# marella/ctransformers

Measured on NVIDIA H100. Metric: decode tokens/s Llama-2-7B Q4_K_M b=1, higher is better.
Workload: dtype int8 (q4_K/q6_K weights x q8_K activations, mma.sync u8 x s8 -> exact int32), fp32 combine in the reference's order

## Files before the change

ctransformers_b200/csrc/engine.cu:

```cuda
#include "engine.cuh"

#include <algorithm>
#include <chrono>
#include <cstdio>
#include <cstring>
#include <stdexcept>

#include "attention.cuh"
#include "matvec.cuh"
#include "prefill.cuh"
#include "repack.cuh"
#include "sample_gpu.cuh"
#include "stream.cuh"
#include "tables.hpp"
#include "tp_nccl.hpp"

namespace ctb {

#define CTB_CUDA(expr)                                                                                         \
  do {                                                                                                         \
    cudaError_t e__ = (expr);                                                                                  \
    if (e__ != cudaSuccess)                                                                                    \
      throw std::runtime_error(std::string("CUDA error: ") + cudaGetErrorString(e__) + " at " + __FILE__ + ":" + \
                               std::to_string(__LINE__) + " (" #expr ")" + watchdog_note());                   \
// ... 19 lines not shown
  int prev = -1;
  explicit DeviceGuard(int dev) {
    cudaGetDevice(&prev);
    if (prev != dev) {
      cudaError_t e = cudaSetDevice(dev);
      if (e != cudaSuccess) throw std::runtime_error(std::string("CUDA error: ") + cudaGetErrorString(e) + " (cudaSetDevice)");
    }
  }
  ~DeviceGuard() { int cur = -1; cudaGetDevice(&cur); if (prev >= 0 && cur != prev) cudaSetDevice(prev); }
};

struct StepOp {
  Phase ph;
  int mvk = 0;
  bool stream = false;
};

__global__ void k_advance(int* state, int* out_tokens) {
  const int t = state[4];
  out_tokens[state[2]] = t;
  state[0] = t;
  state[1] += 1;
  state[2] += 1;
  state[3] = state[1] + 1;
}

struct PrefillState {
  std::vector<void*> bufs;
  PPhase* d_prog = nullptr;
  int n_phases = 0;
// ... 20 lines not shown

size_t engine_arena_bytes(const GGUFFile& g, const HParams& hp) {
  size_t total = 0;
  for (const auto& t : g.tensors) {
    total += align_up(t.nbytes, 256) + 4 * 256;
    if (t.ne[1] > 0) total += align_up(t.nbytes / (size_t)t.ne[1] * ST_ROWS, 256);
  }
  total += UP_CHUNK * UP_BUFS + 256;
  const size_t kv = (size_t)hp.n_layer * (hp.n_ctx + 256) * hp.n_embd_gqa() * 2;
  total += 2 * align_up(kv, 256);
  total += 3 * align_up(65536 * 2, 256);
  total += align_up((size_t)hp.n_ctx * (hp.head_dim() / 2) * 8, 256);
  const size_t qkv = (size_t)hp.n_embd + 2 * (size_t)hp.n_embd_gqa();
  total += 4 * (2 * (size_t)hp.n_embd + qkv + 4 * (size_t)hp.n_embd + 2 * (size_t)hp.n_ff + 2 * (size_t)hp.n_vocab) + 64 * 256 + 8192;
  total += ((size_t)hp.n_layer * 10 + 8) * (sizeof(Phase) * 2 + 2 * 1024) + 8192;
  total += 1 << 20;
  return total;
}

void* Engine::alloc(size_t bytes, size_t align) {
  const size_t off = align_up(arena_used_, align);
  if (off + bytes > arena_size_) throw std::runtime_error("device arena exhausted");
  arena_used_ = off + bytes;
  return arena_ + off;
}

struct Uploader {
  uint8_t* host[UP_BUFS] = {nullptr, nullptr, nullptr};
  uint8_t* dev[UP_BUFS] = {nullptr, nullptr, nullptr};
  cudaEvent_t done[UP_BUFS] = {nullptr, nullptr, nullptr};
// ... 262 lines not shown
  }
  const size_t gqa_l = (size_t)nkv_ * hp_.head_dim(), qw_l = (size_t)nh_ * hp_.head_dim();
  const size_t kv = (size_t)hp_.n_layer * hp_.n_ctx * gqa_l;
  const size_t vv = (size_t)hp_.n_layer * kv_ctx_pad(hp_.n_ctx) * gqa_l;
  kc_ = (uint16_t*)alloc(kv * 2);
  vc_ = (uint16_t*)alloc(vv * 2);
  CTB_CUDA(cudaMemset(kc_, 0, kv * 2));
  CTB_CUDA(cudaMemset(vc_, 0, vv * 2));
  const size_t qkv = qw_l + 2 * gqa_l;
  d_state_ = (int*)alloc(64);
  xa_ = (float*)alloc(hp_.n_embd * 4); xb_ = (float*)alloc(hp_.n_embd * 4);
  qkv_ = (float*)alloc(qkv * 4);
  attn_ = (float*)alloc(hp_.n_embd * 4); attn_o_ = (float*)alloc(hp_.n_embd * 4);
  ffn_ = (float*)alloc((size_t)nff_ * 4);
  ffn2_ = (float*)alloc((size_t)nff_ * 4);
  d_logits_ = (float*)alloc((size_t)hp_.n_vocab * 4);
  d_embd_ = (float*)alloc(hp_.n_embd * 4);
  d_logits_keep_ = (float*)alloc((size_t)hp_.n_vocab * 4);
  d_embd_keep_ = (float*)alloc(hp_.n_embd * 4);
  d_sync_ = (unsigned*)alloc(64);
  CTB_CUDA(cudaMemset(d_state_, 0, 64));
  CTB_CUDA(cudaMemset(d_sync_, 0, 64));
  CTB_CUDA(cudaMallocHost(&h_logits_, (size_t)hp_.n_vocab * 4));
  CTB_CUDA(cudaMallocHost(&h_embd_, (size_t)hp_.n_embd * 4));
  memset(h_logits_, 0, (size_t)hp_.n_vocab * 4);
  memset(h_embd_, 0, (size_t)hp_.n_embd * 4);

  if (const char* e = getenv("CTB_NO_PDL")) pdl_ = !(e[0] == '1');
  if (const char* e = getenv("CTB_NO_SPEC")) spec_on_ = !(e[0] == '1');
  if (const char* e = getenv("CTB_STEP_FUSE")) fused_ = !(e[0] == '0');
// ... 142 lines not shown
    op.ph.em.out = buf; op.ph.em.K = n_embd;
    ops_.push_back(op);
  };
  auto take_input = [&](MVParams& p) {
    if (!xchg_due) return;
    p.x = (const float*)xc_ll_[tp_.rank]; p.x_mode = 2; p.x_parts = tp_.world; p.x_stride = n_embd; p.sum_out = x_sum_into;
  };
  auto mark_exchange = [&](size_t first_op) {
    if (!xchg_due) return;
    if (ops_.size() != first_op + 1) throw std::runtime_error("tensor parallel (fused exchange): the consumer of an exchange must be one mat-vec phase");
    fill_xc(ops_[first_op].ph.xc, 1);
    n_xchg++;
    xchg_due = false; x_sum_into = nullptr;
  };
  const float kq_scale = 1.0f / sqrtf((float)n_embd / (float)hp_.n_head);
  ops_.clear();
  {
    StepOp op{};
    op.ph.kind = PH_EMBED;
    op.ph.em.table = tok_embd_; op.ph.em.row_bytes = tok_row_bytes_; op.ph.em.tokens = d_state_; op.ph.em.out = xa_;
    op.ph.em.type = tok_type_; op.ph.em.K = n_embd; op.ph.em.n_vocab = hp_.n_vocab;
    ops_.push_back(op);
  }
  float* x = xa_;
  float* y = xb_;
  for (int il = 0; il < hp_.n_layer; il++) {
    const LayerW& L = layers_[il];
    uint16_t* kc = kc_ + (size_t)il * hp_.n_ctx * gqa;
    uint16_t* vc = vc_ + (size_t)il * gqa * kv_ctx_pad(hp_.n_ctx);
    AttnParams ap{};
// ... 22 lines not shown
          p.act = act_format_for(ws[i]->type); p.nseg = 0;
          for (int j = i; j < 3; j++)
            if (!done[j] && act_format_for(ws[j]->type) == p.act) { p.seg[p.nseg++] = seg(*ws[j], outs[j]); done[j] = true; }
          push_matvec(p, MVK_QKV);
        }
        mark_exchange(first_op);
      }
      push_attn();
      {
        MVParams p{};
        p.x = attn_; p.norm_mode = NORM_NONE; p.K = qw; p.act = act_format_for(L.wo.type); p.nseg = 1;
        p.seg[0] = (!tp || tp_lead) ? seg(L.wo, y, EPI_ADD, x) : seg(L.wo, y);
        push_matvec(p, MVK_WO);
        if (tp) push_xchg(y);
      }
      {
        MVParams p{};
        p.x = y; p.norm_w = L.ffn_norm; p.norm_mode = NORM_RMS; p.eps = hp_.eps; p.K = n_embd;
        const size_t first_op = ops_.size();
        take_input(p);
        p.act = act_format_for(L.w1.type); p.nseg = 2;
        p.seg[0] = seg(L.w1, ffn_, EPI_SILU); p.seg[1] = seg(L.w3, ffn2_);
        push_matvec(p, MVK_UP);
        mark_exchange(first_op);
      }
      {
        MVParams p{};
        p.x = ffn_; p.x2 = ffn2_; p.x_mode = 1; p.norm_mode = NORM_NONE; p.K = nff_; p.act = act_format_for(L.w2.type); p.nseg = 1;
        p.seg[0] = (!tp || tp_lead) ? seg(L.w2, x, EPI_ADD, y) : seg(L.w2, x);
        push_matvec(p, MVK_DOWN);
        if (tp) push_xchg(x);
      }
    } else {
      const int qkv_w = (hp_.n_head + 2 * n_kv) * hd;
      float* q = qkv_; float* k = qkv_ + (size_t)hp_.n_head * hd; float* v = k + (size_t)n_kv * hd;
      const bool two_norms = L.attn_norm2 != nullptr;
      const bool fuse = !two_norms && act_format_for(L.wqkv.type) == act_format_for(L.w3.type);
      {
        MVParams p{};
        p.x = x; p.norm_mode = NORM_LAYER; p.eps = hp_.eps; p.K = n_embd;
        p.norm_w = two_norms ? L.attn_norm2 : L.attn_norm; p.norm_b = two_norms ? L.attn_norm2_b : L.attn_norm_b;
        p.act = act_format_for(L.wqkv.type); p.nseg = 1;
        p.seg[0] = seg(L.wqkv, qkv_);
        if (fuse) { p.seg[1] = seg(L.w3, ffn_, EPI_GELU); p.nseg = 2; }
        ap.q = q; ap.k = k; ap.v = v; ap.q_stride = qkv_w; ap.kv_stride = qkv_w;
        push_matvec(p, MVK_QKV);
      }
      if (!fuse) {
        MVParams p{};
        p.x = x; p.norm_mode = NORM_LAYER; p.eps = hp_.eps; p.K = n_embd; p.norm_w = L.attn_norm; p.norm_b = L.attn_norm_b;
        p.act = act_format_for(L.w3.type); p.nseg = 1;
        p.seg[0] = seg(L.w3, ffn_, EPI_GELU);
        push_matvec(p, MVK_UP);
      }
      push_attn();
      {
        MVParams p{};
        p.x = attn_; p.norm_mode = NORM_NONE; p.K = n_embd; p.act = act_format_for(L.wo.type); p.nseg = 1;
        p.seg[0] = seg(L.wo, attn_o_);
        push_matvec(p, MVK_WO);
      }
      {
        MVParams p{};
        p.x = ffn_; p.norm_mode = NORM_NONE; p.K = hp_.n_ff; p.act = act_format_for(L.w2.type); p.nseg = 1;
        p.seg[0] = seg(L.w2, y, EPI_ADD2, attn_o_, x);
        push_matvec(p, MVK_DOWN);
      }
      std::swap(x, y);
    }
  }
  n_body_ = (int)ops_.size();
  {
    MVParams p{};
    p.x = x; p.norm_w = out_norm_; p.norm_b = out_norm_b_; p.norm_mode = hp_.falcon ? NORM_LAYER : NORM_RMS; p.eps = hp_.eps; p.K = n_embd;
    const size_t first_op = ops_.size();
    take_input(p);
    p.norm_out = d_embd_; p.act = act_format_for(output_.type); p.nseg = 1;
    p.seg[0] = seg(output_, d_logits_);
    push_matvec(p, MVK_OUT);
    mark_exchange(first_op);

// ... 13 lines not shown
  if (const char* e = getenv("CTB_ST_SLOTS")) {
    const int want = atoi(e);
    if (want >= ST_W && want < step_slots_ && want % ST_W == 0) { step_smem_ -= (size_t)(step_slots_ - want) * ST_SLOT; step_slots_ = want; }
  }
  ring_attn_ = st_attn_ring_ok(hp_.n_ctx, step_slots_) && !getenv("CTB_NO_RING_ATTN");
  for (StepOp& op : ops_) if (op.ph.kind == PH_ATTN) op.ph.q6 = ring_attn_ ? 1 : 0;
  if (any_stream && step_slots_ < ST_W) throw std::runtime_error("model rows are too long for the step kernel's shared memory");
  if (any_stream) CTB_CUDA(step_set_smem_limit(step_smem_));
  else fused_ = false;
  d_prog_ = (Phase*)alloc((ops_.size() + 1) * sizeof(Phase), 256);
  d_prog_mv_ = (Phase*)alloc((ops_.size() + 1) * sizeof(Phase), 256);
  d_bounds_ = (int*)alloc((ops_.size() + 1) * (size_t)(sm_count_ + 1) * 4, 256);
  d_bounds_mv_ = (int*)alloc((ops_.size() + 1) * (size_t)(sm_count_ + 1) * 4, 256);
}

void Engine::upload_prog(Phase* dst, int* dst_bounds, const std::vector<StepOp>& ops) {
  std::vector<Phase> phs(ops.size());
  for (size_t i = 0; i < ops.size(); i++) phs[i] = ops[i].ph;
  CTB_CUDA(cudaMemcpy(dst, phs.data(), phs.size() * sizeof(Phase), cudaMemcpyHostToDevice));
  std::vector<Phase> run = phs;
  for (size_t i = 0; i < ops.size(); i++) if (ops[i].ph.kind == PH_XCHG || (ops[i].ph.kind == PH_MATVEC && !ops[i].stream)) run[i].kind = -1;
  const std::vector<int> b = step_bounds(run.data(), (int)run.size(), sm_count_);
  CTB_CUDA(cudaMemcpy(dst_bounds, b.data(), b.size() * 4, cudaMemcpyHostToDevice));
}

void Engine::enqueue_ops(const std::vector<StepOp>& ops, const Phase* d_prog, const int* d_bounds, int n) {
  launches_per_step_ = 0;
  StepLaunch step_shape_;
  step_shape_.grid = step_grid_; step_shape_.n_slots = step_slots_; step_shape_.smem = step_smem_;
  auto capable = [&](const StepOp& op) { return op.ph.kind != PH_XCHG && (op.ph.kind != PH_MATVEC || op.stream); };
  int i = 0;
  while (i < n) {
    const StepOp& op = ops[i];
// ... 57 lines not shown
  CTB_CUDA(cudaEventCreate(&e));
  CTB_CUDA(cudaEventRecord(e, stream_));
  prof_ev_.push_back(e);
  prof_kind_.push_back(kind);
}

int Engine::profile_step(int token, int n_past, double ms_by_kind[4], int count_by_kind[4]) {
  DeviceGuard dev_guard(device_);
  if (tp_.world > 1) throw std::runtime_error("not available in tensor-parallel mode (every rank must run the same launches)");
  spec_pending_ = false; spec_deferred_ = false; spec_pos_ = -1; spec_streak_ = 0;
  if (h_state_cap_ < 1) { h_state_cap_ = 512; CTB_CUDA(cudaMallocHost(&h_state_, (size_t)h_state_cap_ * 16)); }
  h_state_[0] = token; h_state_[1] = n_past; h_state_[2] = 0; h_state_[3] = n_past + 1;
  CTB_CUDA(cudaMemcpyAsync(d_state_, h_state_, 16, cudaMemcpyHostToDevice, stream_));
  const long keep = launches_per_step_;
  const bool keep_fused = fused_;
  profiling_ = true; fused_ = false;
  try { enqueue_ops(ops_, d_prog_, d_bounds_, n_body_ + 1); } catch (...) { profiling_ = false; fused_ = keep_fused; throw; }
  profiling_ = false; fused_ = keep_fused;
  launches_per_step_ = keep;
  CTB_CUDA(cudaStreamSynchronize(stream_));
  int n = 0;
  for (size_t i = 1; i < prof_ev_.size(); i++) {
    float ms = 0;
    cudaEventElapsedTime(&ms, prof_ev_[i - 1], prof_ev_[i]);
    const int k = prof_kind_[i];
    if (k >= 0 && k < 4) { ms_by_kind[k] += ms; count_by_kind[k]++; n++; }
  }
  for (cudaEvent_t e : prof_ev_) cudaEventDestroy(e);
  prof_ev_.clear(); prof_kind_.clear();
  return n;
}

double Engine::time_matvec_only(int reps, long* launches, unsigned mask) {
  if (!mask) mask = ~0u;
  if (tp_.world > 1) throw std::runtime_error("not available in tensor-parallel mode (every rank must run the same launches)");
  spec_pending_ = false; spec_deferred_ = false; spec_pos_ = -1; spec_streak_ = 0;
  DeviceGuard dev_guard(device_);
  std::vector<StepOp> sel;
  for (int i = 0; i <= n_body_; i++)
    if (ops_[i].ph.kind == PH_MATVEC && ((mask >> ops_[i].mvk) & 1)) sel.push_back(ops_[i]);
  if (sel.empty()) { if (launches) *launches = 0; return 0.0; }
  upload_prog(d_prog_mv_, d_bounds_mv_, sel);
  cudaStream_t user = stream_, cap;
  CTB_CUDA(cudaStreamCreateWithFlags(&cap, cudaStreamNonBlocking));
  const long keep = launches_per_step_;
  cudaGraphExec_t ex = nullptr;
  stream_ = cap;
  try {
    cudaGraph_t g;
    CTB_CUDA(cudaStreamBeginCapture(cap, cudaStreamCaptureModeThreadLocal));
    enqueue_ops(sel, d_prog_mv_, d_bounds_mv_, (int)sel.size());
    CTB_CUDA(cudaStreamEndCapture(cap, &g));
    CTB_CUDA(cudaGraphInstantiate(&ex, g, 0));
    cudaGraphDestroy(g);
  } catch (...) { stream_ = user; launches_per_step_ = keep; cudaStreamDestroy(cap); throw; }
  if (launches) *launches = (long)sel.size();
  stream_ = user; launches_per_step_ = keep;
// ... 46 lines not shown
  graph_full_ = graph_nolog_ = graph_greedy_ = nullptr;
}

void Engine::build_graphs() {
  destroy_graphs();
  if (!d_tokens_out_) {
    tokens_out_cap_ = std::max(hp_.n_ctx, 4096);
    CTB_CUDA(cudaMalloc(&d_tokens_out_, (size_t)tokens_out_cap_ * 4));
    CTB_CUDA(cudaMallocHost(&h_tokens_out_, (size_t)tokens_out_cap_ * 4));
  }
  cudaStream_t user = stream_;
  cudaStream_t cap;
  CTB_CUDA(cudaStreamCreateWithFlags(&cap, cudaStreamNonBlocking));
  stream_ = cap;
  ops_.back().ph.pk.out_tokens = d_tokens_out_;
  upload_prog(d_prog_, d_bounds_, ops_);
  auto capture = [&](bool logits, bool greedy) {
    cudaGraph_t g;
    CTB_CUDA(cudaStreamBeginCapture(cap, cudaStreamCaptureModeThreadLocal));
    enqueue_ops(ops_, d_prog_, d_bounds_, n_body_ + (logits || tp_peer_ ? 1 : 0) + (greedy ? 1 : 0));
    CTB_CUDA(cudaStreamEndCapture(cap, &g));
    cudaGraphExec_t ex;
    CTB_CUDA(cudaGraphInstantiate(&ex, g, 0));
    cudaGraphDestroy(g);
    return ex;
  };
  try {
    graph_nolog_ = capture(false, false);
    graph_greedy_ = capture(true, true);
    graph_full_ = capture(true, false);
  } catch (...) {
// ... 304 lines not shown
```

ctransformers_b200/csrc/engine.cuh:

```cuda
#pragma once
#include <cmath>
#include <memory>
#include <string>
#include <vector>

#include "device_types.cuh"
#include "gguf.hpp"

namespace ctb {

struct TPShard {
  int rank = 0, world = 1;
  int head0 = 0, head1 = 0, kv0 = 0, kv1 = 0, ff0 = 0, ff1 = 0;
  void* comm = nullptr;
};
TPShard tp_shard(int n_embd, int n_head, int n_head_kv, int n_ff, int rank, int world);

struct HParams {
  bool falcon = false;
  int n_vocab = 0, n_ctx_train = 0, n_embd = 0, n_ff = 0, n_head = 0, n_head_kv = 0, n_layer = 0, n_rot = 0;
  float eps = 1e-5f, rope_base = 10000.f, rope_scale = 1.f;
  int n_ctx = 512;
  int head_dim() const { return n_embd / n_head; }
  int n_embd_gqa() const { return head_dim() * n_head_kv; }
// ... 53 lines not shown
  cudaStream_t stream_ = nullptr;
  bool own_stream_ = true;
  uint8_t* arena_ = nullptr;
  size_t arena_size_ = 0, arena_used_ = 0;
  void* alloc(size_t bytes, size_t align = 256);

  DevMat output_;
  const uint8_t* tok_embd_ = nullptr; int tok_type_ = 0; size_t tok_row_bytes_ = 0;
  const float* out_norm_ = nullptr; const float* out_norm_b_ = nullptr;
  std::vector<LayerW> layers_;
  uint16_t *silu_tab_ = nullptr, *gelu_tab_ = nullptr, *exp_tab_ = nullptr;
  float2* rope_ = nullptr;
  uint16_t *kc_ = nullptr, *vc_ = nullptr;
  int* d_state_ = nullptr;
  float *xa_ = nullptr, *xb_ = nullptr, *qkv_ = nullptr, *attn_ = nullptr, *attn_o_ = nullptr, *ffn_ = nullptr, *ffn2_ = nullptr, *d_logits_ = nullptr, *d_embd_ = nullptr, *d_logits_keep_ = nullptr, *d_embd_keep_ = nullptr;
  float *h_logits_ = nullptr, *h_embd_ = nullptr;
  int* h_state_ = nullptr;
  int h_state_cap_ = 0;
  long h_state_next_ = 0;
  int* h_tokens_out_ = nullptr;
  int* d_tokens_out_ = nullptr;
  int tokens_out_cap_ = 0;

  cudaGraphExec_t graph_full_ = nullptr, graph_nolog_ = nullptr, graph_greedy_ = nullptr;
  cudaEvent_t ev0_ = nullptr, ev1_ = nullptr, ev_pick_ = nullptr;
  bool spec_on_ = true, spec_pending_ = false;
  bool spec_deferred_ = false;
  bool sampler_mode_ = false;
  cudaEvent_t ev_sample_ = nullptr;
  void launch_deferred_spec();
// ... 9 lines not shown
  void release();
  DevMat upload_matrix(const GGUFTensor& t, struct Uploader& up, int want_K, int want_M, int row0 = 0, int row1 = -1, int k0 = 0, int k1 = -1);
  const float* upload_vector(const GGUFFile& g, const std::string& name, bool required, int want_n);
  std::vector<StepOp> ops_;
  int n_body_ = 0;
  Phase* d_prog_ = nullptr;
  Phase* d_prog_mv_ = nullptr;
  int *d_bounds_ = nullptr, *d_bounds_mv_ = nullptr;
  unsigned* d_sync_ = nullptr;
  int step_grid_ = 0, step_slots_ = 0;
  size_t step_smem_ = 0;
  bool fused_ = true;
  bool ring_attn_ = false;
  void build_ops();
  void push_matvec(struct MVParams& p, int kind);
  void upload_prog(Phase* dst, int* dst_bounds, const std::vector<StepOp>& ops);
  void enqueue_ops(const std::vector<StepOp>& ops, const Phase* d_prog, const int* d_bounds, int n);
  void build_graphs();
  void destroy_graphs();
  bool eager_ = false;
  bool host_fresh_ = true;
  void host_views();
  struct SampleGpuOut* d_sample_ = nullptr;
  struct SampleGpuOut* h_sample_ = nullptr;
  int* d_last_ = nullptr;
  struct PrefillState* pf_ = nullptr;
  bool prefill_on_ = true;
  int prefill_min_ = 4;
  long prefill_launches_ = 0;
  long single_steps_ = 0;
  bool ensure_prefill();
// ... 15 lines not shown
```

ctransformers_b200/csrc/matvec.cuh:

```cuda
#pragma once
#include "device_types.cuh"
#include "attention.cuh"

namespace ctb {

#ifndef CTB_THREADS
#define CTB_THREADS 512
#endif
constexpr int MV_THREADS = CTB_THREADS;
constexpr int MV_WARPS = MV_THREADS / 32;
constexpr int MV_ROWS = 4;
constexpr int MV_MAX_SEG = 3;

enum : int { NORM_NONE = 0, NORM_RMS = 1, NORM_LAYER = 2 };
enum : int { EPI_STORE = 0, EPI_ADD = 1, EPI_GELU = 2, EPI_ADD2 = 3, EPI_SILU = 4 };

#ifndef ST_WATCHDOG_NS
#define ST_WATCHDOG_NS 4000000000ull
#endif
static __device__ int* g_st_dbg = nullptr;
static __device__ __noinline__ void st_fail(int code, int aux) {
  int* d = g_st_dbg;
  if (d) { d[0] = code; d[1] = (int)blockIdx.x; d[2] = aux; d[3] = (int)threadIdx.x; __threadfence_system(); }
  __trap();
// ... 79 lines not shown
__device__ __forceinline__ double block_sum_f64(double s, double* red ) {
  s = warp_sum(s);
  bar_sync<BAR, NT>();
  if ((threadIdx.x & 31) == 0) red[threadIdx.x >> 5] = s;
  bar_sync<BAR, NT>();
  double t = 0.0;
#pragma unroll
  for (int w = 0; w < NT / 32; w++) t += red[w];
  return t;
}

__device__ __forceinline__ uint32_t pack4(const int* q) {
  return (uint32_t)(q[0] & 0xff) | ((uint32_t)(q[1] & 0xff) << 8) | ((uint32_t)(q[2] & 0xff) << 16) | ((uint32_t)(q[3] & 0xff) << 24);
}

__device__ __forceinline__ void load16_ll(const uint2* p, unsigned epoch, float (&u)[16]) {
  uint4 q[8];
  unsigned long long t0 = 0;
  for (;;) {
    bool ok = true;
#pragma unroll
    for (int j = 0; j < 8; j++) {
      asm volatile("ld.volatile.global.v4.u32 {%0,%1,%2,%3}, [%4];" : "=r"(q[j].x), "=r"(q[j].y), "=r"(q[j].z), "=r"(q[j].w) : "l"(p + 2 * j) : "memory");
    }
#pragma unroll
    for (int j = 0; j < 8; j++) ok &= q[j].y == epoch && q[j].w == epoch;
    if (ok) break;
    if (!t0) t0 = globaltimer_ns();
    else if (globaltimer_ns() - t0 > XC_WATCHDOG_NS) st_fail(10, (int)epoch);
  }
// ... 113 lines not shown
#pragma unroll
      for (int e = 0; e < 16; e++) {
        float y = v[e];
        if (norm_mode == NORM_LAYER) y = __fsub_rn(y, mean);
        y = __fmul_rn(y, scale);
        if (nw) y = __fmul_rn(y, w[e]);
        if (nb_) y = __fadd_rn(y, bb[e]);
        v[e] = y;
      }
    }
    if (write_norm && norm_out && valid > 0) {
#pragma unroll
      for (int e = 0; e < 16; e++) if (e < valid) norm_out[base + e] = v[e];
    }
    if (act == ACT_Q8_K) {
      float amax = 0.f, mx = 0.f;
#pragma unroll
      for (int e = 0; e < 16; e++) { const float ax = fabsf(v[e]); if (ax > amax) { amax = ax; mx = v[e]; } }
      float gmax = amax;
#pragma unroll
      for (int o = 8; o > 0; o >>= 1) gmax = fmaxf(gmax, __shfl_xor_sync(0xffffffffu, gmax, o));
      const unsigned who = __ballot_sync(0xffffffffu, amax == gmax);
      const int hbase = lane & 16, hl = lane & 15;
      const unsigned mine = (who >> hbase) & 0xffffu;
      const float maxv = __shfl_sync(0xffffffffu, mx, hbase + __ffs(mine) - 1);
      if (valid > 0) {
        const int b = base >> 8;
        int q[16];
        int sum = 0;
        if (gmax == 0.f) {
#pragma unroll
          for (int e = 0; e < 16; e++) q[e] = 0;
          if (hl == 0) dd[b] = 0.f;
        } else {
          const float iscale = __fdiv_rn(-128.f, maxv);
#pragma unroll
          for (int e = 0; e < 16; e++) {
            const float val = __fmaf_rn(iscale, v[e], 12582912.f);
            q[e] = min(127, (__float_as_int(val) & 0x007fffff) - 0x00400000);
            sum += q[e];
          }
          if (hl == 0) dd[b] = __fdiv_rn(1.f, iscale);
        }
        bs[b * 16 + hl] = (int16_t)sum;
#pragma unroll
        for (int j = 0; j < 4; j++) {
          const int wi = hl * 4 + j;
          *(uint32_t*)(qs + q8k_word_offset(b, wi >> 3, wi & 7)) = pack4(q + 4 * j);
        }
      }
    } else if (act == ACT_Q8_0) {
      float amax = 0.f;
#pragma unroll
      for (int e = 0; e < 16; e++) amax = fmaxf(amax, fabsf(v[e]));
      amax = fmaxf(amax, __shfl_xor_sync(0xffffffffu, amax, 1));
      if (valid > 0) {
        const float d = __fdiv_rn(amax, 127.f);
        const float id = amax != 0.f ? __fdiv_rn(127.f, amax) : 0.f;
        int q[16];
#pragma unroll
        for (int e = 0; e < 16; e++) q[e] = __float2int_rn(__fmul_rn(v[e], id));
        *(uint4*)(qs + base) = make_uint4(pack4(q), pack4(q + 4), pack4(q + 8), pack4(q + 12));
        if ((lane & 1) == 0) dd[base >> 5] = h2f(f2h(d));
      }
    } else if (act == ACT_F16) {
// ... 179 lines not shown
```

ctransformers_b200/csrc/ops_abi.cu:

```cuda
#include <cmath>
#include <cstdio>
#include <cstring>
#include <functional>
#include <memory>
#include <stdexcept>
#include <string>
#include <vector>

#include "../../include/ctransformers_b200.h"
#include "attention.cuh"
#include "matvec.cuh"
#include "prefill.cuh"
#include "repack.cuh"
#include "stream.cuh"
#include "tables.hpp"

using namespace ctb;

namespace {

#define OPS_CUDA(expr)                                                                                     \
  do {                                                                                                     \
    cudaError_t e__ = (expr);                                                                              \
    if (e__ != cudaSuccess) throw std::runtime_error(std::string("CUDA error: ") + cudaGetErrorString(e__) + " (" #expr ")"); \
// ... 396 lines not shown
    upload(w3, type, w3_blocks, K, M);
    DevBuf dx((size_t)K * 4), dg((size_t)M * 4), du((size_t)M * 4), dy((size_t)M * 4);
    OPS_CUDA(cudaMemcpy(dx.p, x, (size_t)K * 4, cudaMemcpyHostToDevice));
    MVParams p{};
    p.x = dx.as<float>(); p.norm_mode = NORM_NONE; p.K = K; p.act = act_format_for(type); p.nseg = 2;
    p.seg[0].w = w1.m; p.seg[0].out = dg.as<float>(); p.seg[0].epi = EPI_SILU; p.seg[1].w = w3.m; p.seg[1].out = du.as<float>();
    run_matvec(p);
    const size_t smem = (size_t)M * 4 + 64;
    OPS_CUDA(cudaFuncSetAttribute(k_gate_dump, cudaFuncAttributeMaxDynamicSharedMemorySize, (int)std::max<size_t>(smem, 48 * 1024)));
    k_gate_dump<<<1, MV_THREADS, smem>>>(dg.as<float>(), du.as<float>(), tables().silu, M, dy.as<float>());
    OPS_CUDA(cudaGetLastError());
    OPS_CUDA(cudaMemcpy(out, dy.p, (size_t)M * 4, cudaMemcpyDeviceToHost));
  });
}

int ctb_matvec_partition(const int* types, const int* rows, int nseg, int K, int n_sm, int* first_tile, int* meta) {
  if (nseg < 1 || nseg > MV_MAX_SEG || K <= 0 || K % 256 != 0 || n_sm < 1) return -1;
  MVParams p{};
  p.K = K; p.nseg = nseg; p.act = ACT_Q8_K;
  for (int s = 0; s < nseg; s++) {
    if (!type_is_kquant(types[s]) || rows[s] < 1) return -1;
    p.seg[s].w.type = types[s]; p.seg[s].w.K = K; p.seg[s].w.M = rows[s]; p.seg[s].w.nb = K / 256;
  }
  TileSpace ts;
  ts.init(p);
  const int nb = K / 256;
  long max_items = 0;
  for (int c = 0; c <= n_sm; c++) first_tile[c] = ts.boundary(c, n_sm);
  for (int c = 0; c < n_sm; c++) {
    long items = 0;
// ... 26 lines not shown
```

ctransformers_b200/csrc/stream.cuh:

```cuda
#pragma once
#include "matvec.cuh"

namespace ctb {

#ifndef CTB_ST_WARPS
#define CTB_ST_WARPS 10
#endif
constexpr int ST_W = CTB_ST_WARPS;
constexpr int ST_NT = ST_W * 32;
constexpr int ST_THREADS = ST_NT + 32;
constexpr int ST_SLOT = 9216;
#ifndef CTB_ST_DEPTH
#define CTB_ST_DEPTH 2
#endif
constexpr int ST_MAX_DEPTH = CTB_ST_DEPTH;
constexpr int ST_MAX_SLOTS = ST_W * ST_MAX_DEPTH;
constexpr int ST_MAXT = 16;
constexpr int ST_ROWS = 16;
constexpr int ST_BAR = 1;
constexpr int ST_STATE = 6;

__host__ __device__ inline int st_row_block_bytes(int type) { return type == GT_Q4_K ? 144 : (type == GT_Q5_K ? 176 : 210); }
__host__ __device__ inline int st_block_bytes(int type) { return ST_ROWS * st_row_block_bytes(type); }
#ifndef CTB_CHUNK_Q4
// ... 117 lines not shown
  if (threadIdx.x < 64) zero[threadIdx.x] = 0;
  for (int i = threadIdx.x; i < nb * 4; i += NT) {
    const int16_t* b4 = a.bs + (i >> 2) * 16 + 4 * (i & 3);
    const int p0 = (int)b4[0] + (int)b4[1], p1 = (int)b4[2] + (int)b4[3];
    pairs[i] = (uint32_t)(p0 & 0xffff) | ((uint32_t)p1 << 16);
  }
  if (q6) {
    for (int i = threadIdx.x; i < nb * 64; i += NT) {
      const int b = i >> 6, grp = (i >> 3) & 7, l = i & 7;
      const int w = *(const int*)(a.qs + q8k_word_offset(b, grp, l));
      cneg[((b * 4 + (l >> 1)) * 8 + grp) * 2 + (l & 1)] = -32 * __dp4a(0x01010101, w, 0);
    }
  }
  bar_sync<BAR, NT>();
  return s;
}

__device__ __forceinline__ void unpack_k4(uint32_t s0, uint32_t s1, uint32_t s2, uint32_t& sc03, uint32_t& sc47, uint32_t& m03, uint32_t& m47) {
  sc03 = s0 & 0x3f3f3f3fu;
  m03 = s1 & 0x3f3f3f3fu;
  sc47 = (s2 & 0x0f0f0f0fu) | (((s0 >> 6) & 0x03030303u) << 4);
  m47 = ((s2 >> 4) & 0x0f0f0f0fu) | (((s1 >> 6) & 0x03030303u) << 4);
}
__device__ __forceinline__ int pack16(int lo, int hi) { return (int)__byte_perm((uint32_t)lo, (uint32_t)hi, 0x5410); }
__device__ __forceinline__ int scale_fold8(int d0, int d1, int d2, int d3, int d4, int d5, int d6, int d7, uint32_t s03, uint32_t s47) {
  int s = __dp2a_lo(pack16(d0, d1), (int)s03, 0);
  s = __dp2a_hi(pack16(d2, d3), (int)s03, s);
  s = __dp2a_lo(pack16(d4, d5), (int)s47, s);
  s = __dp2a_hi(pack16(d6, d7), (int)s47, s);
  return s;
// ... 281 lines not shown
struct XchgParams {
  int world, rank, index, n;
  int role;
  uint2* ll[XC_MAX_WORLD];
};
struct EmbedParams { const uint8_t* table; size_t row_bytes; const int* tokens; float* out; int type, K, n_vocab; };
struct PickParams { const float* logits; int* state; int* out_tokens; int n; };
struct alignas(16) Phase {
  int kind;
  int q6;
  MVParams mv;
  AttnParams at;
  EmbedParams em;
  PickParams pk;
  XchgParams xc;
};

struct StepArgs {
  const Phase* prog;
  int n_phases;
  int n_slots;
  unsigned* sync;
  const int* bounds;
  unsigned long long* trace;
};

__device__ __forceinline__ unsigned ld_relaxed_u32(const unsigned* p) {
  unsigned v;
  asm volatile("ld.relaxed.gpu.global.u32 %0, [%1];" : "=r"(v) : "l"(p) : "memory");
  return v;
}
// ... 86 lines not shown
  if (warp == (int)((seq0 + (uint32_t)g.n_k) % ST_W)) attn_scores(p.hd, s.k16, 1, 0, 8, s.q16, p.kq_scale, s.sc + g.pos);
  bar_sync<ST_BAR, ST_NT>();
  attn_softmax<ST_NT, ST_BAR>(s.sc, s.p16, g.T, p.exp_tab, red_f, red_d);
  for (int cc = warp; cc < ATTN_CH; cc += ST_W) {
    const int c = cg * ATTN_CH + cc;
    const uint32_t n = seq0 + (uint32_t)(g.n_k + cc / g.cv), slot = st_slot(n, S);
    mbar_wait(&full_bar[slot], st_parity(n, S), 9, (int)n);
    const uint16_t* vrow = (const uint16_t*)(ring + (size_t)slot * ST_SLOT + (size_t)(cc % g.cv) * g.nchv * 512);
    const float o = attn_vp(vrow, s.p16, g, g.pos, s.v16[c]);
    if (lane == 0) p.out[(size_t)h * p.hd + c] = o;
  }
  bar_sync<ST_BAR, ST_NT>();
  if (threadIdx.x < g.n_v) {
    const uint32_t n = seq0 + (uint32_t)(g.n_k + threadIdx.x);
    mbar_arrive(&empty_bar[st_slot(n, S)]);
  }
}

__device__ __forceinline__ void st_producer(const StepArgs& args, uint8_t* ring, uint64_t* full_bar, uint64_t* empty_bar) {
  const int lane = threadIdx.x & 31;
  const uint32_t S = (uint32_t)(args.n_slots / ST_W);
  const uint64_t weight_pol = l2_policy_evict_first();
  uint32_t seq = 0;
  for (int ip = 0; ip < args.n_phases; ip++) {
    const Phase* ph = args.prog + ip;
    if (ph->kind == PH_ATTN) {
      if (ph->q6) st_attn_produce(ph->at, ring, full_bar, empty_bar, S, seq);
      continue;
    }
    if (ph->kind != PH_MATVEC) continue;
// ... 26 lines not shown
        }
        __syncwarp();
        seq += (uint32_t)__popc(mask);
      }
    }
  }
}

template <bool XC>
__device__ __forceinline__ void st_matvec_phase(const Phase& ph, const NormPre& np, uint8_t* ring, uint8_t* act_smem, double* red, uint64_t* full_bar, uint64_t* empty_bar,
                                                float (*mailbox)[ST_STATE * 32], int* flags, uint32_t S, uint32_t& seq, const int* tb, unsigned long long* tr,
                                                unsigned xc_base) {
  const MVParams& p = ph.mv;
  const int warp = threadIdx.x >> 5, lane = threadIdx.x & 31;
  const unsigned epoch = XC ? xc_base + (unsigned)ph.xc.index + 1u : 0u;
  stage_activation<ST_NT, ST_BAR, XC>(p, np, p.norm_w, p.norm_b, p.norm_out, p.norm_mode, p.eps, p.K, ACT_Q8_K, act_smem, red, blockIdx.x == 0, epoch);
  StAct a = st_act_extras<ST_NT, ST_BAR>(act_smem, p.K, ph.q6 != 0);
  a.xc = XC && ph.xc.role == 2 ? &ph.xc : nullptr;
  a.epoch = epoch;
  if (tr && threadIdx.x == 0) tr[1] = globaltimer_ns();
  bool first_item = tr != nullptr && threadIdx.x == 0;
  TileSpace ts;
  ts.init(p);
  const int nb = p.K >> 8;
  const int T0 = tb[0], T1 = tb[1];
#pragma unroll 1
  for (int w0 = T0; w0 < T1; w0 += ST_MAXT) {
    if (w0 != T0) {
      bar_sync<ST_BAR, ST_NT>();
      if (threadIdx.x < ST_MAXT) flags[threadIdx.x] = 0;
      bar_sync<ST_BAR, ST_NT>();
// ... 17 lines not shown
        const int b0 = kc * kb, nblk = min(kb, nb - b0);
        const MVSeg& sg = p.seg[seg];
        const uint8_t* sp = ring + (size_t)slot * ST_SLOT;
        mbar_wait(&full_bar[slot], st_parity(n, S), 5, (int)n);
        if (first_item) { tr[2] = globaltimer_ns(); first_item = false; }
        volatile float* mail = mailbox[j];
        volatile int* flag = flags + j;
        const bool last = kc == nch - 1;
        if (type == GT_Q4_K) run_item<GT_Q4_K, XC>(sp, &empty_bar[slot], nblk, b0, kc, last, a, lane, mail, flag, sg, p, til * ST_ROWS);
        else if (type == GT_Q6_K) run_item<GT_Q6_K, XC>(sp, &empty_bar[slot], nblk, b0, kc, last, a, lane, mail, flag, sg, p, til * ST_ROWS);
        else run_item<GT_Q5_K, XC>(sp, &empty_bar[slot], nblk, b0, kc, last, a, lane, mail, flag, sg, p, til * ST_ROWS);
      }
      seq += (uint32_t)cnt;
    }
  }
}

__device__ __forceinline__ void st_pick_phase(const PickParams& pk, float* bv, int* bi) {
  float best = -INFINITY;
  int idx = 0x7fffffff;
  for (int i = threadIdx.x; i < pk.n; i += ST_NT) {
    const float v = __ldcg(pk.logits + i);
    if (v > best) { best = v; idx = i; }
  }
#pragma unroll
  for (int o = 16; o > 0; o >>= 1) {
    const float ov = __shfl_xor_sync(0xffffffffu, best, o);
    const int oi = __shfl_xor_sync(0xffffffffu, idx, o);
    if (ov > best || (ov == best && oi < idx)) { best = ov; idx = oi; }
  }
// ... 200 lines not shown
```

ctransformers_b200/lib.py:

```python
import ctypes as C
from pathlib import Path
from typing import Optional

LIB_DIR = Path(__file__).resolve().parent / "lib"
LIB_NAME = "libctransformers.so"


class ConfigStruct(C.Structure):
    _fields_ = [("context_length", C.c_int), ("gpu_layers", C.c_int), ("mmap", C.c_bool), ("mlock", C.c_bool)]


def find_library(path: Optional[str] = None) -> str:
    if path:
        return str(path)
    lib = LIB_DIR / LIB_NAME
    if not lib.is_file():
        raise OSError(
            f"{lib} has not been built. Build it with `python -m ctransformers_b200.build` "
            "(needs nvcc; compiles for sm_90a). There is no CPU fallback library."
        )
    return str(lib)


_P = C.c_void_p
# ... 34 lines not shown
    "ctb_tp_shard": (C.c_int, [C.c_int, C.c_int, C.c_int, C.c_int, C.c_int, C.c_int, _IP]),
    "ctb_llm_decode_greedy": (C.c_double, [_P, C.c_int, C.c_int, C.c_int, _IP]),
    "ctb_llm_profile_step": (C.c_int, [_P, C.c_int, C.c_int, C.POINTER(C.c_double), _IP]),
    "ctb_llm_time_matvec_only": (C.c_double, [_P, C.c_int, C.POINTER(C.c_long)]),
    "ctb_llm_time_matvec_kinds": (C.c_double, [_P, C.c_int, C.POINTER(C.c_long), C.c_uint]),
    "ctb_mul_mat": (C.c_int, [C.c_int, _P, _P, _P, C.c_int, C.c_int, C.c_int]),
    "ctb_quantize_row_q8_K": (C.c_int, [_P, _P, C.c_int]),
    "ctb_quantize_row_q8_0": (C.c_int, [_P, _P, C.c_int]),
    "ctb_norm": (C.c_int, [C.c_int, _P, _P, _P, _P, C.c_int, C.c_float]),
    "ctb_rope": (C.c_int, [_P, C.c_int, C.c_int, C.c_int, C.c_int, C.c_float, C.c_float]),
    "ctb_attention": (C.c_int, [_P, _P, _P, _P, C.c_int, C.c_int, C.c_int, C.c_int, C.c_int, C.c_float]),
    "ctb_attention_path": (C.c_int, [C.c_int, _P, _P, _P, _P, _P, _P, C.c_int, C.c_int, C.c_int, C.c_int, C.c_int, C.c_int, _P, C.c_int,
                                     C.c_float, C.c_float]),
    "ctb_llm_paths": (C.c_long, [_P, _IP, C.c_int]),
    "ctb_ffn_gate": (C.c_int, [C.c_int, _P, _P, _P, _P, C.c_int, C.c_int]),
    "ctb_matvec_partition": (C.c_int, [_IP, _IP, C.c_int, C.c_int, C.c_int, _IP, _IP]),
    "ctb_get_row": (C.c_int, [C.c_int, _P, C.c_int, C.c_int, C.c_int, _P]),
    "ctb_vocab_load": (_P, [C.c_char_p]),
    "ctb_vocab_free": (None, [_P]),
    "ctb_vocab_size": (C.c_int, [_P]),
    "ctb_vocab_tokenize": (C.c_int, [_P, C.c_char_p, C.c_bool, _IP, C.c_int]),
    "ctb_vocab_piece": (C.c_int, [_P, C.c_int, C.c_char_p, C.c_int]),
    "ctb_sample": (C.c_int, [_FP, C.c_int, _IP, C.c_int, C.c_int, C.c_float, C.c_float, C.c_float, C.c_int]),
}


def load_library(path: Optional[str] = None):
    lib = C.CDLL(find_library(path))
    for table, required in ((PROTOTYPES, True), (EXTRA_PROTOTYPES, False)):
        for name, (res, args) in table.items():
# ... 9 lines not shown
```

include/ctransformers_b200.h:

```cpp
#ifndef CTRANSFORMERS_B200_H_
#define CTRANSFORMERS_B200_H_

#include <stdbool.h>
#include <stddef.h>
#include <stdint.h>

#ifdef __cplusplus
extern "C" {
#endif

typedef struct LLM LLM;

typedef struct ctransformers_config {
  int context_length;
  int gpu_layers;
  bool mmap;
  bool mlock;
} ctransformers_config;

LLM* ctransformers_llm_create(const char* model_path, const char* model_type, const ctransformers_config config);
void ctransformers_llm_delete(LLM* llm);
int ctransformers_llm_tokenize(LLM* llm, const char* text, const bool add_bos_token, int* output);
const char* ctransformers_llm_detokenize(LLM* llm, const int token);
bool ctransformers_llm_is_eos_token(LLM* llm, const int token);
// ... 40 lines not shown
int ctb_vocab_piece(ctb_vocab* v, int token, char* buf, int cap);
int ctb_sample(const float* logits, int n_vocab, const int* last_tokens, int n_last, int top_k, float top_p, float temperature,
               float repetition_penalty, int seed);

int ctb_mul_mat(int type, const void* w_blocks, const float* x, float* dst, int K, int M, int N);
int ctb_quantize_row_q8_K(const float* x, void* y, int k);
int ctb_quantize_row_q8_0(const float* x, void* y, int k);
int ctb_norm(int mode, const float* x, const float* w, const float* b, float* y, int n, float eps);
int ctb_rope(float* x, int n_heads, int head_dim, int pos, int mode, float freq_base, float freq_scale);
int ctb_attention(const float* q, const uint16_t* kcache, const uint16_t* vcache, float* out, int n_head, int n_kv, int head_dim,
                  int T, int n_total, float kq_scale);
int ctb_attention_path(int path, const float* q, const float* k_new, const float* v_new, uint16_t* kcache, uint16_t* vcache,
                       float* out, int n_head, int n_kv, int head_dim, int n_ctx, int pos0, int n_tok, const int* n_total,
                       int rope_mode, float freq_base, float kq_scale);
int ctb_ffn_gate(int type, const void* w1_blocks, const void* w3_blocks, const float* x, float* out, int K, int M);
int ctb_matvec_partition(const int* types, const int* rows, int nseg, int K, int n_sm, int* first_tile, int* meta);

int ctb_get_row(int type, const void* table_blocks, int K, int n_rows, int row, float* out);

#ifdef __cplusplus
}
#endif
#endif
```

Measured before the change: 354.2.

## Publish quantized FFN activation image from up-projection for down-projection reuse

```diff
diff --git a/ctransformers_b200/csrc/engine.cu b/ctransformers_b200/csrc/engine.cu
--- a/ctransformers_b200/csrc/engine.cu
+++ b/ctransformers_b200/csrc/engine.cu
@@ -57,6 +57,8 @@
   Phase ph;
   int mvk = 0;
   bool stream = false;
+  int pub_src = 0, pub_dst = 0;
+  Q8KPub pub{};
 };
 
 __global__ void k_advance(int* state, int* out_tokens) {
@@ -107,6 +109,7 @@
   const size_t qkv = (size_t)hp.n_embd + 2 * (size_t)hp.n_embd_gqa();
   total += 4 * (2 * (size_t)hp.n_embd + qkv + 4 * (size_t)hp.n_embd + 2 * (size_t)hp.n_ff + 2 * (size_t)hp.n_vocab) + 64 * 256 + 8192;
   total += ((size_t)hp.n_layer * 10 + 8) * (sizeof(Phase) * 2 + 2 * 1024) + 8192;
+  total += q8k_image_bytes(hp.n_ff) + (size_t)hp.n_ff / 64 + 3 * 256;
   total += 1 << 20;
   return total;
 }
@@ -399,6 +402,11 @@
   attn_ = (float*)alloc(hp_.n_embd * 4); attn_o_ = (float*)alloc(hp_.n_embd * 4);
   ffn_ = (float*)alloc((size_t)nff_ * 4);
   ffn2_ = (float*)alloc((size_t)nff_ * 4);
+  {
+    ffn_q8_ = (uint8_t*)alloc(q8k_image_bytes(nff_));
+    ffn_q8_cnt_ = (unsigned*)alloc((size_t)(nff_ / 256 + 1) * 4);
+    CTB_CUDA(cudaMemset(ffn_q8_cnt_, 0, (size_t)(nff_ / 256 + 1) * 4));
+  }
   d_logits_ = (float*)alloc((size_t)hp_.n_vocab * 4);
   d_embd_ = (float*)alloc(hp_.n_embd * 4);
   d_logits_keep_ = (float*)alloc((size_t)hp_.n_vocab * 4);
@@ -571,6 +579,13 @@
     xchg_due = false; x_sum_into = nullptr;
   };
   const float kq_scale = 1.0f / sqrtf((float)n_embd / (float)hp_.n_head);
+  int n_pub = 0;
+  auto publish = [&](uint8_t* img, unsigned* cnt, const float* px, const float* px2, int K, int n, int segs) {
+    StepOp& op = ops_.back();
+    op.pub_src = ++n_pub;
+    op.pub.img = img; op.pub.cnt = cnt; op.pub.x = px; op.pub.x2 = px2; op.pub.K = K; op.pub.n = n; op.pub.segs = segs;
+    return n_pub;
+  };
   ops_.clear();
   {
     StepOp op{};
@@ -623,6 +638,7 @@
         push_matvec(p, MVK_WO);
         if (tp) push_xchg(y);
       }
+      int ffn_pub;
       {
         MVParams p{};
         p.x = y; p.norm_w = L.ffn_norm; p.norm_mode = NORM_RMS; p.eps = hp_.eps; p.K = n_embd;
@@ -631,6 +647,7 @@
         p.act = act_format_for(L.w1.type); p.nseg = 2;
         p.seg[0] = seg(L.w1, ffn_, EPI_SILU); p.seg[1] = seg(L.w3, ffn2_);
         push_matvec(p, MVK_UP);
+        ffn_pub = publish(ffn_q8_, ffn_q8_cnt_, ffn_, ffn2_, nff_, 2 * 256 / ST_ROWS, 3);
         mark_exchange(first_op);
       }
       {
@@ -638,6 +655,7 @@
         p.x = ffn_; p.x2 = ffn2_; p.x_mode = 1; p.norm_mode = NORM_NONE; p.K = nff_; p.act = act_format_for(L.w2.type); p.nseg = 1;
         p.seg[0] = (!tp || tp_lead) ? seg(L.w2, x, EPI_ADD, y) : seg(L.w2, x);
         push_matvec(p, MVK_DOWN);
+        ops_.back().pub_dst = ffn_pub;
         if (tp) push_xchg(x);
       }
     } else {
@@ -655,12 +673,14 @@
         ap.q = q; ap.k = k; ap.v = v; ap.q_stride = qkv_w; ap.kv_stride = qkv_w;
         push_matvec(p, MVK_QKV);
       }
+      int ffn_pub = fuse ? publish(ffn_q8_, ffn_q8_cnt_, ffn_, nullptr, nff_, 256 / ST_ROWS, 2) : 0;
       if (!fuse) {
         MVParams p{};
         p.x = x; p.norm_mode = NORM_LAYER; p.eps = hp_.eps; p.K = n_embd; p.norm_w = L.attn_norm; p.norm_b = L.attn_norm_b;
         p.act = act_format_for(L.w3.type); p.nseg = 1;
         p.seg[0] = seg(L.w3, ffn_, EPI_GELU);
         push_matvec(p, MVK_UP);
+        ffn_pub = publish(ffn_q8_, ffn_q8_cnt_, ffn_, nullptr, nff_, 256 / ST_ROWS, 1);
       }
       push_attn();
       {
@@ -674,6 +694,7 @@
         p.x = ffn_; p.norm_mode = NORM_NONE; p.K = hp_.n_ff; p.act = act_format_for(L.w2.type); p.nseg = 1;
         p.seg[0] = seg(L.w2, y, EPI_ADD2, attn_o_, x);
         push_matvec(p, MVK_DOWN);
+        ops_.back().pub_dst = ffn_pub;
       }
       std::swap(x, y);
     }
@@ -717,9 +738,25 @@
   d_bounds_mv_ = (int*)alloc((ops_.size() + 1) * (size_t)(sm_count_ + 1) * 4, 256);
 }
 
-void Engine::upload_prog(Phase* dst, int* dst_bounds, const std::vector<StepOp>& ops) {
+void Engine::upload_prog(Phase* dst, int* dst_bounds, const std::vector<StepOp>& ops, bool fused) {
   std::vector<Phase> phs(ops.size());
   for (size_t i = 0; i < ops.size(); i++) phs[i] = ops[i].ph;
+  if (fused) {
+    auto in_step = [](const StepOp& op) { return op.ph.kind == PH_MATVEC && op.stream; };
+    for (size_t i = 0; i < ops.size(); i++) {
+      if (!ops[i].pub_src || !in_step(ops[i])) continue;
+      const Q8KPub& pb = ops[i].pub;
+      bool ok = pb.K % 256 == 0;
+      for (int s = 0; s < ops[i].ph.mv.nseg; s++) ok &= !((pb.segs >> s) & 1) || ops[i].ph.mv.seg[s].w.M == pb.K;
+      for (size_t j = i + 1; j < ops.size() && ok; j++) {
+        const StepOp& c = ops[j];
+        if (c.pub_dst != ops[i].pub_src || !in_step(c)) continue;
+        if (c.ph.mv.K != pb.K || c.ph.mv.x != pb.x || (c.ph.mv.x_mode == 1 ? c.ph.mv.x2 : nullptr) != pb.x2 || c.ph.mv.x_mode == 2) continue;
+        phs[i].pub = pb;
+        phs[j].x_img = pb.img;
+      }
+    }
+  }
   CTB_CUDA(cudaMemcpy(dst, phs.data(), phs.size() * sizeof(Phase), cudaMemcpyHostToDevice));
   std::vector<Phase> run = phs;
   for (size_t i = 0; i < ops.size(); i++) if (ops[i].ph.kind == PH_XCHG || (ops[i].ph.kind == PH_MATVEC && !ops[i].stream)) run[i].kind = -1;
@@ -807,8 +844,9 @@
   CTB_CUDA(cudaMemcpyAsync(d_state_, h_state_, 16, cudaMemcpyHostToDevice, stream_));
   const long keep = launches_per_step_;
   const bool keep_fused = fused_;
+  upload_prog(d_prog_mv_, d_bounds_mv_, ops_, false);
   profiling_ = true; fused_ = false;
-  try { enqueue_ops(ops_, d_prog_, d_bounds_, n_body_ + 1); } catch (...) { profiling_ = false; fused_ = keep_fused; throw; }
+  try { enqueue_ops(ops_, d_prog_mv_, d_bounds_mv_, n_body_ + 1); } catch (...) { profiling_ = false; fused_ = keep_fused; throw; }
   profiling_ = false; fused_ = keep_fused;
   launches_per_step_ = keep;
   CTB_CUDA(cudaStreamSynchronize(stream_));
@@ -833,7 +871,7 @@
   for (int i = 0; i <= n_body_; i++)
     if (ops_[i].ph.kind == PH_MATVEC && ((mask >> ops_[i].mvk) & 1)) sel.push_back(ops_[i]);
   if (sel.empty()) { if (launches) *launches = 0; return 0.0; }
-  upload_prog(d_prog_mv_, d_bounds_mv_, sel);
+  upload_prog(d_prog_mv_, d_bounds_mv_, sel, fused_);
   cudaStream_t user = stream_, cap;
   CTB_CUDA(cudaStreamCreateWithFlags(&cap, cudaStreamNonBlocking));
   const long keep = launches_per_step_;
@@ -910,7 +948,7 @@
   CTB_CUDA(cudaStreamCreateWithFlags(&cap, cudaStreamNonBlocking));
   stream_ = cap;
   ops_.back().ph.pk.out_tokens = d_tokens_out_;
-  upload_prog(d_prog_, d_bounds_, ops_);
+  upload_prog(d_prog_, d_bounds_, ops_, fused_);
   auto capture = [&](bool logits, bool greedy) {
     cudaGraph_t g;
     CTB_CUDA(cudaStreamBeginCapture(cap, cudaStreamCaptureModeThreadLocal));
diff --git a/ctransformers_b200/csrc/engine.cuh b/ctransformers_b200/csrc/engine.cuh
--- a/ctransformers_b200/csrc/engine.cuh
+++ b/ctransformers_b200/csrc/engine.cuh
@@ -91,6 +91,8 @@
   uint16_t *kc_ = nullptr, *vc_ = nullptr;
   int* d_state_ = nullptr;
   float *xa_ = nullptr, *xb_ = nullptr, *qkv_ = nullptr, *attn_ = nullptr, *attn_o_ = nullptr, *ffn_ = nullptr, *ffn2_ = nullptr, *d_logits_ = nullptr, *d_embd_ = nullptr, *d_logits_keep_ = nullptr, *d_embd_keep_ = nullptr;
+  uint8_t* ffn_q8_ = nullptr;
+  unsigned* ffn_q8_cnt_ = nullptr;
   float *h_logits_ = nullptr, *h_embd_ = nullptr;
   int* h_state_ = nullptr;
   int h_state_cap_ = 0;
@@ -130,7 +132,7 @@
   bool ring_attn_ = false;
   void build_ops();
   void push_matvec(struct MVParams& p, int kind);
-  void upload_prog(Phase* dst, int* dst_bounds, const std::vector<StepOp>& ops);
+  void upload_prog(Phase* dst, int* dst_bounds, const std::vector<StepOp>& ops, bool fused);
   void enqueue_ops(const std::vector<StepOp>& ops, const Phase* d_prog, const int* d_bounds, int n);
   void build_graphs();
   void destroy_graphs();
diff --git a/ctransformers_b200/csrc/matvec.cuh b/ctransformers_b200/csrc/matvec.cuh
--- a/ctransformers_b200/csrc/matvec.cuh
+++ b/ctransformers_b200/csrc/matvec.cuh
@@ -117,6 +117,43 @@
   return (uint32_t)(q[0] & 0xff) | ((uint32_t)(q[1] & 0xff) << 8) | ((uint32_t)(q[2] & 0xff) << 16) | ((uint32_t)(q[3] & 0xff) << 24);
 }
 
+__device__ __forceinline__ void q8k_quantize16(const float (&v)[16], bool store, int b, int8_t* qs, float* dd, int16_t* bs) {
+  const int lane = threadIdx.x & 31;
+  float amax = 0.f, mx = 0.f;
+#pragma unroll
+  for (int e = 0; e < 16; e++) { const float ax = fabsf(v[e]); if (ax > amax) { amax = ax; mx = v[e]; } }
+  float gmax = amax;
+#pragma unroll
+  for (int o = 8; o > 0; o >>= 1) gmax = fmaxf(gmax, __shfl_xor_sync(0xffffffffu, gmax, o));
+  const unsigned who = __ballot_sync(0xffffffffu, amax == gmax);
+  const int hbase = lane & 16, hl = lane & 15;
+  const unsigned mine = (who >> hbase) & 0xffffu;
+  const float maxv = __shfl_sync(0xffffffffu, mx, hbase + __ffs(mine) - 1);
+  if (!store) return;
+  int q[16];
+  int sum = 0;
+  if (gmax == 0.f) {
+#pragma unroll
+    for (int e = 0; e < 16; e++) q[e] = 0;
+    if (hl == 0) dd[b] = 0.f;
+  } else {
+    const float iscale = __fdiv_rn(-128.f, maxv);
+#pragma unroll
+    for (int e = 0; e < 16; e++) {
+      const float val = __fmaf_rn(iscale, v[e], 12582912.f);
+      q[e] = min(127, (__float_as_int(val) & 0x007fffff) - 0x00400000);
+      sum += q[e];
+    }
+    if (hl == 0) dd[b] = __fdiv_rn(1.f, iscale);
+  }
+  bs[b * 16 + hl] = (int16_t)sum;
+#pragma unroll
+  for (int j = 0; j < 4; j++) {
+    const int wi = hl * 4 + j;
+    *(uint32_t*)(qs + q8k_word_offset(b, wi >> 3, wi & 7)) = pack4(q + 4 * j);
+  }
+}
+
 __device__ __forceinline__ void load16_ll(const uint2* p, unsigned epoch, float (&u)[16]) {
   uint4 q[8];
   unsigned long long t0 = 0;
@@ -260,41 +297,7 @@
       for (int e = 0; e < 16; e++) if (e < valid) norm_out[base + e] = v[e];
     }
     if (act == ACT_Q8_K) {
-      float amax = 0.f, mx = 0.f;
-#pragma unroll
-      for (int e = 0; e < 16; e++) { const float ax = fabsf(v[e]); if (ax > amax) { amax = ax; mx = v[e]; } }
-      float gmax = amax;
-#pragma unroll
-      for (int o = 8; o > 0; o >>= 1) gmax = fmaxf(gmax, __shfl_xor_sync(0xffffffffu, gmax, o));
-      const unsigned who = __ballot_sync(0xffffffffu, amax == gmax);
-      const int hbase = lane & 16, hl = lane & 15;
-      const unsigned mine = (who >> hbase) & 0xffffu;
-      const float maxv = __shfl_sync(0xffffffffu, mx, hbase + __ffs(mine) - 1);
-      if (valid > 0) {
-        const int b = base >> 8;
-        int q[16];
-        int sum = 0;
-        if (gmax == 0.f) {
-#pragma unroll
-          for (int e = 0; e < 16; e++) q[e] = 0;
-          if (hl == 0) dd[b] = 0.f;
-        } else {
-          const float iscale = __fdiv_rn(-128.f, maxv);
-#pragma unroll
-          for (int e = 0; e < 16; e++) {
-            const float val = __fmaf_rn(iscale, v[e], 12582912.f);
-            q[e] = min(127, (__float_as_int(val) & 0x007fffff) - 0x00400000);
-            sum += q[e];
-          }
-          if (hl == 0) dd[b] = __fdiv_rn(1.f, iscale);
-        }
-        bs[b * 16 + hl] = (int16_t)sum;
-#pragma unroll
-        for (int j = 0; j < 4; j++) {
-          const int wi = hl * 4 + j;
-          *(uint32_t*)(qs + q8k_word_offset(b, wi >> 3, wi & 7)) = pack4(q + 4 * j);
-        }
-      }
+      q8k_quantize16(v, valid > 0, base >> 8, qs, dd, bs);
     } else if (act == ACT_Q8_0) {
       float amax = 0.f;
 #pragma unroll
diff --git a/ctransformers_b200/csrc/ops_abi.cu b/ctransformers_b200/csrc/ops_abi.cu
--- a/ctransformers_b200/csrc/ops_abi.cu
+++ b/ctransformers_b200/csrc/ops_abi.cu
@@ -434,6 +434,29 @@
   });
 }
 
+int ctb_ffn_gate_q8k(int type1, int type3, const void* w1_blocks, const void* w3_blocks, const float* x, void* image, int K, int M) {
+  return guarded("ctb_ffn_gate_q8k", [&] {
+    if (!type_is_kquant(type1) || !type_is_kquant(type3) || K % 256 || M % 256 || M <= 0) throw std::runtime_error("needs K-quant weights and K, M multiples of 256");
+    OwnedMat w1, w3;
+    upload(w1, type1, w1_blocks, K, M);
+    upload(w3, type3, w3_blocks, K, M);
+    const size_t ib = q8k_image_bytes(M);
+    DevBuf dx((size_t)K * 4), dg((size_t)M * 4), du((size_t)M * 4), dimg(ib), dcnt((size_t)M / 256 * 4);
+    OPS_CUDA(cudaMemcpy(dx.p, x, (size_t)K * 4, cudaMemcpyHostToDevice));
+    OPS_CUDA(cudaMemset(dimg.p, 0, ib));
+    OPS_CUDA(cudaMemset(dcnt.p, 0, (size_t)M / 256 * 4));
+    MVParams p{};
+    p.x = dx.as<float>(); p.norm_mode = NORM_NONE; p.K = K; p.act = ACT_Q8_K; p.nseg = 2;
+    p.seg[0].w = w1.m; p.seg[0].out = dg.as<float>(); p.seg[0].epi = EPI_SILU; p.seg[1].w = w3.m; p.seg[1].out = du.as<float>();
+    p.silu_tab = tables().silu; p.gelu_tab = tables().gelu;
+    Phase ph = matvec_phase(p);
+    ph.pub.img = dimg.as<uint8_t>(); ph.pub.cnt = dcnt.as<unsigned>(); ph.pub.x = dg.as<float>(); ph.pub.x2 = du.as<float>();
+    ph.pub.K = M; ph.pub.n = 2 * 256 / ST_ROWS; ph.pub.segs = 3;
+    run_phases({ph});
+    OPS_CUDA(cudaMemcpy(image, dimg.p, ib, cudaMemcpyDeviceToHost));
+  });
+}
+
 int ctb_matvec_partition(const int* types, const int* rows, int nseg, int K, int n_sm, int* first_tile, int* meta) {
   if (nseg < 1 || nseg > MV_MAX_SEG || K <= 0 || K % 256 != 0 || n_sm < 1) return -1;
   MVParams p{};
diff --git a/ctransformers_b200/csrc/stream.cuh b/ctransformers_b200/csrc/stream.cuh
--- a/ctransformers_b200/csrc/stream.cuh
+++ b/ctransformers_b200/csrc/stream.cuh
@@ -155,6 +155,50 @@
   }
   bar_sync<BAR, NT>();
   return s;
+}
+
+struct Q8KPub {
+  uint8_t* img;
+  unsigned* cnt;
+  const float* x;
+  const float* x2;
+  int K;
+  int n;
+  int segs;
+};
+__host__ __device__ inline size_t q8k_image_bytes(int K) { return (((size_t)K + 15) & ~(size_t)15) + q8k_d_bytes(K) + (size_t)(K / 16) * 2; }
+
+static __device__ __noinline__ void q8k_count(const Q8KPub* pb, int b, int c, bool active) {
+  const int lane = threadIdx.x & 31;
+  unsigned old = 0;
+  if (active) asm volatile("atom.acq_rel.gpu.global.add.u32 %0, [%1], %2;" : "=r"(old) : "l"(pb->cnt + b), "r"((unsigned)c) : "memory");
+  for (unsigned m = __ballot_sync(0xffffffffu, active && ((old + (unsigned)c) & (unsigned)(pb->n - 1)) == 0u); m; m &= m - 1) {
+    const int bb = __shfl_sync(0xffffffffu, b, __ffs(m) - 1);
+    const bool mine = lane < 16;
+    float v[16];
+    if (mine) {
+      const int base = bb * 256 + lane * 16;
+      load16<true>(pb->x + base, 16, v);
+      if (pb->x2) {
+        float u[16];
+        load16<true>(pb->x2 + base, 16, u);
+#pragma unroll
+        for (int e = 0; e < 16; e++) v[e] = __fmul_rn(v[e], u[e]);
+      }
+    } else {
+#pragma unroll
+      for (int e = 0; e < 16; e++) v[e] = 0.f;
+    }
+    const size_t off = ((size_t)pb->K + 15) & ~(size_t)15;
+    q8k_quantize16(v, mine, bb, (int8_t*)pb->img, (float*)(pb->img + off), (int16_t*)(pb->img + off + q8k_d_bytes(pb->K)));
+  }
+}
+
+template <int NT, int BAR>
+__device__ __forceinline__ void st_copy_image(const uint8_t* img, uint8_t* smem, int K) {
+  const int n = (int)q8k_image_bytes(K);
+  for (int o = threadIdx.x * 16; o < n; o += NT * 16) *(uint4*)(smem + o) = __ldcg((const uint4*)(img + o));
+  bar_sync<BAR, NT>();
 }
 
 __device__ __forceinline__ void unpack_k4(uint32_t s0, uint32_t s1, uint32_t s2, uint32_t& sc03, uint32_t& sc47, uint32_t& m03, uint32_t& m47) {
@@ -466,7 +510,10 @@
   EmbedParams em;
   PickParams pk;
   XchgParams xc;
+  Q8KPub pub;
+  const uint8_t* x_img;
 };
+static_assert(sizeof(Phase) <= 64 * 16, "k_step fetches a phase descriptor with at most 64 16-byte copies");
 
 struct StepArgs {
   const Phase* prog;
@@ -583,6 +630,27 @@
   if (threadIdx.x < g.n_v) {
     const uint32_t n = seq0 + (uint32_t)(g.n_k + threadIdx.x);
     mbar_arrive(&empty_bar[st_slot(n, S)]);
+  }
+}
+
+__device__ __forceinline__ void st_matvec_count(const Q8KPub* pb, const TileSpace& ts, int T0, int T1) {
+  bar_sync<ST_BAR, ST_NT>();
+  if (threadIdx.x >= 32) return;
+  constexpr int TPB = 256 / ST_ROWS;
+  int base = 0;
+#pragma unroll
+  for (int s = 0; s < MV_MAX_SEG; s++) {
+    if (s < ts.nseg && ((pb->segs >> s) & 1)) {
+      const int a = max(T0, base) - base, e = min(T1, base + ts.tiles[s]) - base;
+      if (a < e) {
+        const int b0 = a / TPB, nblk = (e - 1) / TPB - b0 + 1;
+        for (int i0 = 0; i0 < nblk; i0 += 32) {
+          const int b = b0 + i0 + (int)threadIdx.x;
+          q8k_count(pb, b, min(e, (b + 1) * TPB) - max(a, b * TPB), i0 + (int)threadIdx.x < nblk);
+        }
+      }
+    }
+    base += ts.tiles[s];
   }
 }
 
@@ -639,7 +707,8 @@
   const MVParams& p = ph.mv;
   const int warp = threadIdx.x >> 5, lane = threadIdx.x & 31;
   const unsigned epoch = XC ? xc_base + (unsigned)ph.xc.index + 1u : 0u;
-  stage_activation<ST_NT, ST_BAR, XC>(p, np, p.norm_w, p.norm_b, p.norm_out, p.norm_mode, p.eps, p.K, ACT_Q8_K, act_smem, red, blockIdx.x == 0, epoch);
+  if (ph.x_img) st_copy_image<ST_NT, ST_BAR>(ph.x_img, act_smem, p.K);
+  else stage_activation<ST_NT, ST_BAR, XC>(p, np, p.norm_w, p.norm_b, p.norm_out, p.norm_mode, p.eps, p.K, ACT_Q8_K, act_smem, red, blockIdx.x == 0, epoch);
   StAct a = st_act_extras<ST_NT, ST_BAR>(act_smem, p.K, ph.q6 != 0);
   a.xc = XC && ph.xc.role == 2 ? &ph.xc : nullptr;
   a.epoch = epoch;
@@ -687,6 +756,7 @@
       seq += (uint32_t)cnt;
     }
   }
+  if (ph.pub.img) st_matvec_count(&ph.pub, ts, T0, T1);
 }
 
 __device__ __forceinline__ void st_pick_phase(const PickParams& pk, float* bv, int* bi) {
diff --git a/ctransformers_b200/lib.py b/ctransformers_b200/lib.py
--- a/ctransformers_b200/lib.py
+++ b/ctransformers_b200/lib.py
@@ -72,6 +72,7 @@
                                      C.c_float, C.c_float]),
     "ctb_llm_paths": (C.c_long, [_P, _IP, C.c_int]),
     "ctb_ffn_gate": (C.c_int, [C.c_int, _P, _P, _P, _P, C.c_int, C.c_int]),
+    "ctb_ffn_gate_q8k": (C.c_int, [C.c_int, C.c_int, _P, _P, _P, _P, C.c_int, C.c_int]),
     "ctb_matvec_partition": (C.c_int, [_IP, _IP, C.c_int, C.c_int, C.c_int, _IP, _IP]),
     "ctb_get_row": (C.c_int, [C.c_int, _P, C.c_int, C.c_int, C.c_int, _P]),
     "ctb_vocab_load": (_P, [C.c_char_p]),
diff --git a/include/ctransformers_b200.h b/include/ctransformers_b200.h
--- a/include/ctransformers_b200.h
+++ b/include/ctransformers_b200.h
@@ -78,6 +78,7 @@
                        float* out, int n_head, int n_kv, int head_dim, int n_ctx, int pos0, int n_tok, const int* n_total,
                        int rope_mode, float freq_base, float kq_scale);
 int ctb_ffn_gate(int type, const void* w1_blocks, const void* w3_blocks, const float* x, float* out, int K, int M);
+int ctb_ffn_gate_q8k(int type1, int type3, const void* w1_blocks, const void* w3_blocks, const float* x, void* image, int K, int M);
 int ctb_matvec_partition(const int* types, const int* rows, int nseg, int K, int n_sm, int* first_tile, int* meta);
 
 int ctb_get_row(int type, const void* table_blocks, int K, int n_rows, int row, float* out);
```

Measured after the change: 363.2, median of 6. +2.5%, better.
